# tyui592/Real_Time_Helmet_Detection

Measured on AMD Instinct MI355X. Metric: train imgs/sec, higher is better.
Workload: dtype bf16; 1 GPU; model=hourglass-1-ch128, global_batch=16, imsize=512, parallelism=dp1, engine=hip, fp8=False, hipgraph=True

## Files before the change

### real_time_helmet_detection_amd/ops/csrc/bindings.cpp

```cpp
#include <torch/extension.h>

namespace rthd {
torch::Tensor add_act_fwd(torch::Tensor a, torch::Tensor b, int64_t act);
torch::Tensor add_act_bwd(torch::Tensor dy, torch::Tensor y, int64_t act);

std::vector<torch::Tensor> pool2x2_fwd(torch::Tensor x, bool is_max,
                                       bool need_arg);
torch::Tensor pool2x2_bwd(torch::Tensor dy, torch::Tensor arg, bool is_max,
                          int64_t H, int64_t W);
std::vector<torch::Tensor> maxpool_same_fwd(torch::Tensor x, int64_t k,
                                            bool need_arg);
torch::Tensor maxpool_same_bwd(torch::Tensor dy, torch::Tensor arg,
                               int64_t k);

torch::Tensor upsample2x_add_fwd(torch::Tensor x,
                                 c10::optional<torch::Tensor> skip);
torch::Tensor upsample2x_bwd(torch::Tensor dy);

std::vector<torch::Tensor> centernet_loss_fwd(
    torch::Tensor phm, torch::Tensor poff, torch::Tensor psize,
    torch::Tensor ghm, torch::Tensor goff, torch::Tensor gsize,
    torch::Tensor mask, double alpha, double beta);
std::vector<torch::Tensor> centernet_loss_bwd(
    torch::Tensor phm, torch::Tensor poff, torch::Tensor psize,
    torch::Tensor ghm, torch::Tensor goff, torch::Tensor gsize,
    torch::Tensor mask, torch::Tensor sums, torch::Tensor gout,
    double alpha, double beta);
std::vector<torch::Tensor> centernet_loss_fused_fwd(
    torch::Tensor out, torch::Tensor ghm, torch::Tensor goff,
    torch::Tensor gsize, torch::Tensor mask, double alpha, double beta,
    bool sig_os);
torch::Tensor centernet_loss_fused_bwd(
    torch::Tensor out, torch::Tensor ghm, torch::Tensor goff,
    torch::Tensor gsize, torch::Tensor mask, torch::Tensor sums,
    torch::Tensor glosses, double alpha, double beta, bool sig_os);

std::vector<torch::Tensor> decode_fwd(torch::Tensor hm, torch::Tensor off,
                                      torch::Tensor wh, int64_t scale_factor,
                                      int64_t topk, int64_t pool_size,
                                      bool normalized);
std::vector<torch::Tensor> decode_logits(torch::Tensor out,
                                         int64_t scale_factor, int64_t topk,
                                         int64_t pool_size, bool normalized,
                                         bool flip);
torch::Tensor nms_fwd(torch::Tensor boxes, torch::Tensor scores,
                      double iou_threshold);
std::vector<torch::Tensor> nms_batched(torch::Tensor boxes,
                                       torch::Tensor scores,
                                       double iou_threshold,
                                       double conf_th);
std::vector<torch::Tensor> soft_nms_fwd(torch::Tensor boxes,
                                        torch::Tensor scores, double sigma,
                                        double score_th);
std::vector<torch::Tensor> soft_nms_batched(torch::Tensor boxes,
                                            torch::Tensor scores,
                                            double sigma, double score_th,
                                            double conf_th);

torch::Tensor pack_weights(torch::Tensor w, bool swap, bool to_bf16);
std::vector<torch::Tensor> pack_weights_pair(torch::Tensor w,
                                             bool to_bf16_fwd,
                                             bool to_bf16_dgrad);
torch::Tensor pack_weights_fp8(torch::Tensor w);
torch::Tensor conv_fwd_fp8r(torch::Tensor x, torch::Tensor wpk,
                            torch::Tensor scale, torch::Tensor shift,
                            c10::optional<torch::Tensor> skip,
                            int64_t KH, int64_t KW, int64_t stride,
                            int64_t pad, int64_t Cout, int64_t act,
                            bool out_fp8);
torch::Tensor conv_fwd(torch::Tensor x, torch::Tensor wpk,
                       torch::Tensor scale, torch::Tensor shift,
                       c10::optional<torch::Tensor> skip,
                       int64_t KH, int64_t KW, int64_t stride, int64_t pad,
                       int64_t Cout, int64_t act);
torch::Tensor conv_fwd_small(torch::Tensor x, torch::Tensor wpk,
                             torch::Tensor scale, torch::Tensor shift,
                             c10::optional<torch::Tensor> skip,
                             int64_t KH, int64_t KW, int64_t stride,
                             int64_t pad, int64_t Cout, int64_t act,
                             int64_t splitk);
torch::Tensor conv_fwd_k64(torch::Tensor x, torch::Tensor wpk,
                           torch::Tensor scale, torch::Tensor shift,
                           c10::optional<torch::Tensor> skip,
                           int64_t KH, int64_t KW, int64_t stride,
                           int64_t pad, int64_t Cout, int64_t act);
torch::Tensor stem_im2col(torch::Tensor x, int64_t KS, int64_t stride,
                          int64_t pad);
torch::Tensor wgrad(torch::Tensor x, torch::Tensor dy, int64_t KH,
                    int64_t KW, int64_t stride, int64_t pad);
torch::Tensor wgrad_bf16_fast(torch::Tensor x, torch::Tensor dy, int64_t KH,
                              int64_t KW, int64_t stride, int64_t pad,
                              const std::string& variant);
torch::Tensor lds_tr16_selftest();
std::string wgrad_bf16_choice(int64_t Cin, int64_t Cout, int64_t M);
int64_t wgrad_bf16_chunk_len(int64_t Cin, int64_t Cout, int64_t taps,
                             int64_t M);

std::vector<torch::Tensor> conv_fwd_stats(
    torch::Tensor x, torch::Tensor wpk, torch::Tensor scale,
    torch::Tensor shift, int64_t KH, int64_t KW, int64_t stride,
    int64_t pad, int64_t Cout, int64_t act);
std::vector<torch::Tensor> bn_stats_from_parts(
    torch::Tensor p1, torch::Tensor p2,
    c10::optional<torch::Tensor> running_mean,
    c10::optional<torch::Tensor> running_var,
    double momentum, double eps, int64_t M);
std::vector<torch::Tensor> bn_stats(torch::Tensor x,
                                    c10::optional<torch::Tensor> running_mean,
                                    c10::optional<torch::Tensor> running_var,
                                    double momentum, double eps);
torch::Tensor bn_act_fwd(torch::Tensor x, torch::Tensor mean,
                         torch::Tensor rstd, torch::Tensor gamma,
                         torch::Tensor beta, int64_t act,
                         c10::optional<torch::Tensor> skip);
std::vector<torch::Tensor> bn_act_bwd(torch::Tensor dy, torch::Tensor x,
                                      torch::Tensor mean, torch::Tensor rstd,
                                      torch::Tensor gamma, torch::Tensor beta,
                                      int64_t act,
                                      c10::optional<torch::Tensor> skip);
torch::Tensor col_sum(torch::Tensor x);

std::vector<torch::Tensor> encode_targets(torch::Tensor boxes,
                                          torch::Tensor labels, int64_t H,
                                          int64_t W, int64_t scale_factor,
                                          int64_t num_cls, bool normalized);
torch::Tensor normalize_u8(torch::Tensor img_u8, torch::Tensor table);
int64_t encode_chunk();
torch::Tensor augment_u8(torch::Tensor img_u8, torch::Tensor sizes,
                         torch::Tensor coef, int64_t T,
                         c10::optional<torch::Tensor> table);
}

PYBIND11_MODULE(TORCH_EXTENSION_NAME, m) {
  m.def("add_act_fwd", &rthd::add_act_fwd);
  m.def("add_act_bwd", &rthd::add_act_bwd);
  m.def("pool2x2_fwd", &rthd::pool2x2_fwd);
  m.def("pool2x2_bwd", &rthd::pool2x2_bwd);
  m.def("maxpool_same_fwd", &rthd::maxpool_same_fwd);
  m.def("maxpool_same_bwd", &rthd::maxpool_same_bwd);
  m.def("upsample2x_add_fwd", &rthd::upsample2x_add_fwd);
  m.def("upsample2x_bwd", &rthd::upsample2x_bwd);
  m.def("centernet_loss_fwd", &rthd::centernet_loss_fwd);
  m.def("centernet_loss_bwd", &rthd::centernet_loss_bwd);
  m.def("centernet_loss_fused_fwd", &rthd::centernet_loss_fused_fwd);
  m.def("centernet_loss_fused_bwd", &rthd::centernet_loss_fused_bwd);
  m.def("decode_fwd", &rthd::decode_fwd);
  m.def("decode_logits", &rthd::decode_logits);
  m.def("nms_fwd", &rthd::nms_fwd);
  m.def("nms_batched", &rthd::nms_batched);
  m.def("soft_nms", &rthd::soft_nms_fwd);
  m.def("soft_nms_batched", &rthd::soft_nms_batched);
  m.def("pack_weights",&rthd::pack_weights);
  m.def("pack_weights_pair", &rthd::pack_weights_pair);
  m.def("pack_weights_fp8", &rthd::pack_weights_fp8);
  m.def("conv_fwd_fp8r", &rthd::conv_fwd_fp8r);
  m.def("conv_fwd", &rthd::conv_fwd);
  m.def("conv_fwd_small", &rthd::conv_fwd_small);
  m.def("conv_fwd_k64", &rthd::conv_fwd_k64);
  m.def("stem_im2col", &rthd::stem_im2col);
  m.def("wgrad", &rthd::wgrad);
  m.def("wgrad_bf16_fast", &rthd::wgrad_bf16_fast,
        py::arg("x"), py::arg("dy"), py::arg("kh"), py::arg("kw"),
        py::arg("stride"), py::arg("pad"), py::arg("variant") = "");
  m.def("lds_tr16_selftest", &rthd::lds_tr16_selftest);
  m.def("wgrad_bf16_choice", &rthd::wgrad_bf16_choice);
  m.def("wgrad_bf16_chunk_len", &rthd::wgrad_bf16_chunk_len);
  m.def("conv_fwd_stats", &rthd::conv_fwd_stats);
  m.def("bn_stats_from_parts", &rthd::bn_stats_from_parts,
        py::arg("p1"), py::arg("p2"), py::arg("running_mean") = py::none(),
        py::arg("running_var") = py::none(), py::arg("momentum") = 0.1,
        py::arg("eps") = 1e-5, py::arg("m") = 1);
  m.def("bn_stats", &rthd::bn_stats);
  m.def("bn_act_fwd", &rthd::bn_act_fwd, py::arg("x"), py::arg("mean"), py::arg("rstd"), py::arg("gamma"), py::arg("beta"), py::arg("act"), py::arg("skip") = py::none());
  m.def("bn_act_bwd", &rthd::bn_act_bwd, py::arg("dy"), py::arg("x"), py::arg("mean"), py::arg("rstd"), py::arg("gamma"), py::arg("beta"), py::arg("act"), py::arg("skip") = py::none());
  m.def("col_sum", &rthd::col_sum);
  m.def("encode_targets", &rthd::encode_targets);
  m.def("normalize_u8", &rthd::normalize_u8);
  m.def("encode_chunk", &rthd::encode_chunk);
  m.def("augment_u8", &rthd::augment_u8, py::arg("img_u8"), py::arg("sizes"),
        py::arg("coef"), py::arg("T"), py::arg("table") = py::none());
}

namespace rthd {

static torch::Tensor maxpool2x2_op(torch::Tensor x) {
  return pool2x2_fwd(std::move(x), true, false)[0];
}
static torch::Tensor avgpool2x2_op(torch::Tensor x) {
  return pool2x2_fwd(std::move(x), false, false)[0];
}
static torch::Tensor maxpool_same_op(torch::Tensor x, int64_t k) {
  return maxpool_same_fwd(std::move(x), k, false)[0];
}
static std::tuple<torch::Tensor, torch::Tensor> nms_batched_op(
    torch::Tensor boxes, torch::Tensor scores, double iou, double conf) {
  auto v = nms_batched(std::move(boxes), std::move(scores), iou, conf);
  return {v[0], v[1]};
}
static std::tuple<torch::Tensor, torch::Tensor> soft_nms_op(
    torch::Tensor boxes, torch::Tensor scores, double sigma,
    double score_th) {
  auto v = soft_nms_fwd(std::move(boxes), std::move(scores), sigma, score_th);
  return {v[0], v[1]};
}
static std::tuple<torch::Tensor, torch::Tensor, torch::Tensor>
soft_nms_batched_op(torch::Tensor boxes, torch::Tensor scores, double sigma,
                    double score_th, double conf) {
  auto v = soft_nms_batched(std::move(boxes), std::move(scores), sigma,
                            score_th, conf);
  return {v[0], v[1], v[2]};
}
static std::tuple<torch::Tensor, torch::Tensor, torch::Tensor> decode_op(
    torch::Tensor hm, torch::Tensor off, torch::Tensor wh,
    int64_t scale_factor, int64_t topk, int64_t pool_size, bool normalized) {
  auto v = decode_fwd(std::move(hm), std::move(off), std::move(wh),
                      scale_factor, topk, pool_size, normalized);
  return {v[0], v[1], v[2]};
}
static std::tuple<torch::Tensor, torch::Tensor, torch::Tensor>
decode_logits_op(torch::Tensor out, int64_t scale_factor, int64_t topk,
                 int64_t pool_size, bool normalized, bool flip) {
  auto v = decode_logits(std::move(out), scale_factor, topk, pool_size,
                         normalized, flip);
  return {v[0], v[1], v[2]};
}

}

TORCH_LIBRARY(rthd, m) {
  m.def("conv_fwd(Tensor x, Tensor wpk, Tensor scale, Tensor shift, "
        "Tensor? skip, int kh, int kw, int stride, int pad, int cout, "
        "int act) -> Tensor");
  m.def("conv_fwd_fp8r(Tensor x, Tensor wpk, Tensor scale, Tensor shift, "
        "Tensor? skip, int kh, int kw, int stride, int pad, int cout, "
        "int act, bool out_fp8) -> Tensor");
  m.def("add_act_fwd(Tensor a, Tensor b, int act) -> Tensor");
  m.def("maxpool2x2(Tensor x) -> Tensor");
  m.def("avgpool2x2(Tensor x) -> Tensor");
  m.def("maxpool_same(Tensor x, int k) -> Tensor");
  m.def("upsample2x_add(Tensor x, Tensor? skip) -> Tensor");
  m.def("nms(Tensor boxes, Tensor scores, float iou) -> Tensor");
  m.def("nms_batched(Tensor boxes, Tensor scores, float iou, float conf) "
        "-> (Tensor, Tensor)");
  m.def("soft_nms(Tensor boxes, Tensor scores, float sigma, "
        "float score_th) -> (Tensor, Tensor)");
  m.def("soft_nms_batched(Tensor boxes, Tensor scores, float sigma, "
        "float score_th, float conf) -> (Tensor, Tensor, Tensor)");
  m.def("decode(Tensor hm, Tensor off, Tensor wh, int scale_factor, "
        "int topk, int pool_size, bool normalized) "
        "-> (Tensor, Tensor, Tensor)");
  m.def("decode_logits(Tensor out, int scale_factor, int topk, "
        "int pool_size, bool normalized, bool flip) "
        "-> (Tensor, Tensor, Tensor)");
  m.def("stem_im2col(Tensor x, int ks, int stride, int pad) -> Tensor");
}

TORCH_LIBRARY_IMPL(rthd, CUDA, m) {
  m.impl("conv_fwd", rthd::conv_fwd);
  m.impl("conv_fwd_fp8r", rthd::conv_fwd_fp8r);
  m.impl("add_act_fwd", rthd::add_act_fwd);
  m.impl("maxpool2x2", rthd::maxpool2x2_op);
  m.impl("avgpool2x2", rthd::avgpool2x2_op);
  m.impl("maxpool_same", rthd::maxpool_same_op);
  m.impl("upsample2x_add", rthd::upsample2x_add_fwd);
  m.impl("nms", rthd::nms_fwd);
  m.impl("nms_batched", rthd::nms_batched_op);
  m.impl("soft_nms", rthd::soft_nms_op);
  m.impl("soft_nms_batched", rthd::soft_nms_batched_op);
  m.impl("decode", rthd::decode_op);
  m.impl("decode_logits", rthd::decode_logits_op);
  m.impl("stem_im2col", rthd::stem_im2col);
}
```

### real_time_helmet_detection_amd/ops/csrc/conv.hip

```cpp
#include <mutex>
#include <type_traits>
#include <unordered_map>

#include "conv_common.h"

namespace rthd {



struct PackSrc {
  const float* w;
  int Cout, Cin, KH, KW;
  int64_t s0, s1, s2, s3;
};

template <typename T>
DEV_INLINE void pack_weight_elem(const PackSrc& a, T* __restrict__ pk,
                                 int64_t i, int Rows, int Rp, int Kp,
                                 int swap) {
  const int t = i / ((int64_t)Rp * Kp);
  const int row = (i / Kp) % Rp;
  const int k = i % Kp;
  float v = 0.f;
  const int Kdim = swap ? a.Cout : a.Cin;
// ... 81 lines not shown
        dim3(256), 0, s, pack_src(wc), pk.data_ptr<float>(), g.Rows, g.Rp,
        g.Kp, swap ? 1 : 0);
  HIP_CHECK_LAST();
  return pk;
}

std::vector<torch::Tensor> pack_weights_pair(torch::Tensor w,
                                             bool to_bf16_fwd,
                                             bool to_bf16_dgrad) {
  auto wc = w.to(at::kFloat);
  const PackGeo gf = pack_geo(wc, false), gd = pack_geo(wc, true);
  auto pk = pack_alloc(wc, gf, to_bf16_fwd);
  auto pkt = pack_alloc(wc, gd, to_bf16_dgrad);
  auto s = at::cuda::getCurrentCUDAStream();
  const dim3 grid(ew_grid(gf.n + gd.n, 256));
  auto launch = [&](auto* pf, auto* pd) {
    using TF = std::remove_pointer_t<decltype(pf)>;
    using TD = std::remove_pointer_t<decltype(pd)>;
    hipLaunchKernelGGL((pack_weights_pair_kernel<TF, TD>), grid, dim3(256),
        0, s, pack_src(wc), pf, pd, gf.Rp, gf.Kp, gd.Rp, gd.Kp);
  };
  bf16* fb = reinterpret_cast<bf16*>(pk.data_ptr());
  bf16* db = reinterpret_cast<bf16*>(pkt.data_ptr());
  float* ff = reinterpret_cast<float*>(pk.data_ptr());
  float* df = reinterpret_cast<float*>(pkt.data_ptr());
  if (to_bf16_fwd && to_bf16_dgrad) launch(fb, db);
  else if (to_bf16_fwd) launch(fb, df);
  else if (to_bf16_dgrad) launch(ff, db);
  else launch(ff, df);
  HIP_CHECK_LAST();
  return {pk, pkt};
}


DEV_INLINE int lds_off_f32(int row, int k) {
  return row * 128 + ((k ^ (row & 15)) << 2);
}

template <bool HAS_SKIP, bool STATS = false>
__global__ __launch_bounds__(256)
void conv_fwd_bf16_kernel(const bf16* __restrict__ x,
                          const bf16* __restrict__ wpk,
                          const float* __restrict__ scale,
                          const float* __restrict__ shift,
                          const bf16* __restrict__ skip,
                          const bf16* __restrict__ zpage,
                          bf16* __restrict__ y,
                          ConvGeo g, int act,
                          float* __restrict__ sp1 = nullptr,
                          float* __restrict__ sp2 = nullptr) {
  const int mblk = blockIdx.x;
  const int nblk = blockIdx.y;
  const int tid = threadIdx.x;
  const int lane = tid & 63;
  const int wid = tid >> 6;
  const int wr = wid >> 1, wc = wid & 1;

  extern __shared__ __attribute__((aligned(16))) char smem[];
  char* lds = smem;

  f32x4 acc[4][4] = {};

  const int st_row = tid >> 2;
  const int st_k8 = tid & 3;
  const int k8s0 = st_k8 ^ ((st_row >> 2) & 3);
  const int k8s1 = st_k8 ^ (((st_row + 64) >> 2) & 3);
  const int wbase = wid * 1024;

  int am[2], ab[2], ay[2], ax[2];
#pragma unroll
  for (int h = 0; h < 2; ++h) {
    am[h] = mblk * 128 + st_row + 64 * h;
    pixel_decompose(am[h], g, &ab[h], &ay[h], &ax[h]);
  }

  const int kc = g.Cinp / 32;
  const int taps = g.KH * g.KW;
  const int nsteps = taps * kc;

  int is_step = 0;
  int is_t = 0, is_kb = 0;
  const bf16* aptr[2];
  const bf16* bptr[2];
  bool avalid[2];
  auto tap_setup = [&]() {
    const int dy_ = is_t / g.KW - g.pad;
    const int dx_ = is_t % g.KW - g.pad;
#pragma unroll
    for (int h = 0; h < 2; ++h) {
      const int iy = ay[h] * g.stride + dy_;
      const int ix = ax[h] * g.stride + dx_;
      avalid[h] = am[h] < g.M && iy >= 0 && iy < g.H && ix >= 0 &&
                  ix < g.W;
      const int c0 = (h ? k8s1 : k8s0) * 8;
      aptr[h] = avalid[h]
          ? x + (((int64_t)ab[h] * g.H + iy) * g.W + ix) * g.Cin + c0
          : zpage;
    }
    bptr[0] = wpk + ((int64_t)is_t * g.Coutp + nblk * 128 + st_row) *
        g.Cinp + k8s0 * 8;
    bptr[1] = wpk + ((int64_t)is_t * g.Coutp + nblk * 128 + st_row + 64) *
        g.Cinp + k8s1 * 8;
  };
  tap_setup();

  auto issue_step = [&]() {
    char* base = lds + (is_step % 3) * 16384;
    const int cb = is_kb * 32;
    const bf16* a0 = (avalid[0] && cb + k8s0 * 8 < g.Cin) ? aptr[0] + cb
                                                          : zpage;
    const bf16* a1 = (avalid[1] && cb + k8s1 * 8 < g.Cin) ? aptr[1] + cb
                                                          : zpage;
    __builtin_amdgcn_global_load_lds((glb_void*)a0,
        (lds_void*)(base + wbase), 16, 0, 0);
    __builtin_amdgcn_global_load_lds((glb_void*)a1,
        (lds_void*)(base + 4096 + wbase), 16, 0, 0);
    __builtin_amdgcn_global_load_lds((glb_void*)(bptr[0] + cb),
        (lds_void*)(base + 8192 + wbase), 16, 0, 0);
    __builtin_amdgcn_global_load_lds((glb_void*)(bptr[1] + cb),
        (lds_void*)(base + 12288 + wbase), 16, 0, 0);
    ++is_step;
    if (++is_kb == kc) {
      is_kb = 0;
      if (++is_t < taps) tap_setup();
    }
  };

  issue_step();
  if (nsteps > 1) {
    issue_step();
    asm volatile("s_waitcnt vmcnt(%0)" ::"i"(4) : "memory");
  } else {
    asm volatile("s_waitcnt vmcnt(%0)" ::"i"(0) : "memory");
  }
  __builtin_amdgcn_s_barrier();

  for (int step = 0; step < nsteps; ++step) {
    char* A = lds + (step % 3) * 16384;
    char* B = A + 8192;
    if (step + 2 < nsteps) issue_step();

    const int arow_base = wr * 64 + (lane & 15);
    const int brow_base = wc * 64 + (lane & 15);
    const int k8 = lane >> 4;
    bf16x8 afrag[4], bfrag[4];
#pragma unroll
    for (int i = 0; i < 4; ++i) {
      afrag[i] = *reinterpret_cast<const bf16x8*>(
          A + lds_off_row64(arow_base + 16 * i, k8));
      bfrag[i] = *reinterpret_cast<const bf16x8*>(
          B + lds_off_row64(brow_base + 16 * i, k8));
    }
    asm volatile("s_setprio 1");
#pragma unroll
    for (int mi = 0; mi < 4; ++mi)
#pragma unroll
      for (int ni = 0; ni < 4; ++ni)
        acc[mi][ni] = __builtin_amdgcn_mfma_f32_16x16x32_bf16(
            afrag[mi], bfrag[ni], acc[mi][ni], 0, 0, 0);
    asm volatile("s_setprio 0");

    if (step + 2 < nsteps + 1) {
      if (step + 2 < nsteps)
        asm volatile("s_waitcnt vmcnt(%0)" ::"i"(4) : "memory");
      else
        asm volatile("s_waitcnt vmcnt(%0)" ::"i"(0) : "memory");
    }
    __builtin_amdgcn_s_barrier();
  }

  conv_epilogue<4, 4, HAS_SKIP, STATS>(
      acc, mblk * 128 + wr * 64, nblk * 128 + wc * 64 + (lane & 15), lane,
      g.M, g.Cout, scale, shift, skip, y, act, sp1, sp2,
      (int64_t)mblk * 2 + wr);
}

template <bool HAS_SKIP>
__global__ __launch_bounds__(256)
void conv_fwd_f32_kernel(const float* __restrict__ x,
                         const float* __restrict__ wpk,
                         const float* __restrict__ scale,
                         const float* __restrict__ shift,
                         const float* __restrict__ skip,
                         float* __restrict__ y,
                         ConvGeo g, int act) {
  const int mblk = blockIdx.x;
  const int nblk = blockIdx.y;
  const int tid = threadIdx.x;
  const int lane = tid & 63;
  const int wid = tid >> 6;
  const int wr = wid >> 1, wc = wid & 1;

  extern __shared__ __attribute__((aligned(16))) char smem[];
  float* ldsA = reinterpret_cast<float*>(smem);
  float* ldsB = reinterpret_cast<float*>(smem + 16384);

  f32x4 acc[4][4] = {};

  const int st_row = tid >> 2;
  const int st_k8 = (tid & 3) * 8;

  int am[2], ab[2], ayy[2], axx[2];
#pragma unroll
  for (int h = 0; h < 2; ++h) {
    am[h] = mblk * 128 + st_row + 64 * h;
    pixel_decompose(am[h], g, &ab[h], &ayy[h], &axx[h]);
  }

  const int nsteps = g.KH * g.KW * (g.Cinp / 32);
  const int kc_per_tap = g.Cinp / 32;

  for (int step = 0; step < nsteps; ++step) {
    const int t = step / kc_per_tap;
    const int kb = step % kc_per_tap;
    const int dy = t / g.KW - g.pad;
    const int dx = t % g.KW - g.pad;
    float* A = ldsA;
    float* B = ldsB;
    __syncthreads();

#pragma unroll
    for (int h = 0; h < 2; ++h) {
      const int iy = ayy[h] * g.stride + dy;
      const int ix = axx[h] * g.stride + dx;
      const int c0 = kb * 32 + st_k8;
      float v[8] = {};
      if (am[h] < g.M && iy >= 0 && iy < g.H && ix >= 0 && ix < g.W &&
          c0 < g.Cin) {
        const float* src =
            x + (((int64_t)ab[h] * g.H + iy) * g.W + ix) * g.Cin + c0;
#pragma unroll
        for (int e = 0; e < 8; ++e)
          v[e] = (c0 + e < g.Cin) ? src[e] : 0.f;
      }
#pragma unroll
      for (int e = 0; e < 8; ++e) {
        *reinterpret_cast<float*>(
            reinterpret_cast<char*>(A) +
            lds_off_f32(st_row + 64 * h, st_k8 + e)) = v[e];
      }
    }
#pragma unroll
    for (int h = 0; h < 2; ++h) {
      const int row = st_row + 64 * h;
      const int64_t src_off =
          ((int64_t)t * g.Coutp + nblk * 128 + row) * g.Cinp + kb * 32 +
          st_k8;
#pragma unroll
      for (int e = 0; e < 8; ++e) {
        *reinterpret_cast<float*>(
            reinterpret_cast<char*>(B) + lds_off_f32(row, st_k8 + e)) =
            wpk[src_off + e];
      }
    }

    __syncthreads();

    const int arow = wr * 64 + (lane & 15);
    const int brow = wc * 64 + (lane & 15);
    const int kl = lane >> 4;
#pragma unroll
    for (int ks = 0; ks < 8; ++ks) {
      float afrag[4], bfrag[4];
#pragma unroll
      for (int i = 0; i < 4; ++i) {
        afrag[i] = *reinterpret_cast<const float*>(
            reinterpret_cast<char*>(A) +
            lds_off_f32(arow + 16 * i, ks * 4 + kl));
        bfrag[i] = *reinterpret_cast<const float*>(
            reinterpret_cast<char*>(B) +
            lds_off_f32(brow + 16 * i, ks * 4 + kl));
      }
#pragma unroll
      for (int mi = 0; mi < 4; ++mi)
#pragma unroll
        for (int ni = 0; ni < 4; ++ni)
          acc[mi][ni] = __builtin_amdgcn_mfma_f32_16x16x4f32(
              afrag[mi], bfrag[ni], acc[mi][ni], 0, 0, 0);
    }

    __syncthreads();
  }

  conv_epilogue<4, 4, HAS_SKIP, false>(
      acc, mblk * 128 + wr * 64, nblk * 128 + wc * 64 + (lane & 15), lane,
      g.M, g.Cout, scale, shift, skip, y, act, nullptr, nullptr, 0);
}


const bf16* zero_page_bf16(const torch::Tensor& like) {
  static std::mutex mu;
  static std::unordered_map<int, torch::Tensor> pages;
  const int dev = like.device().index();
  std::lock_guard<std::mutex> lk(mu);
  auto it = pages.find(dev);
  if (it == pages.end())
    it = pages.emplace(dev, torch::zeros({8},
        like.options().dtype(at::kBFloat16))).first;
  return reinterpret_cast<const bf16*>(it->second.data_ptr());
}

namespace {

struct ConvChoice { int small; int splitk; };

std::mutex g_conv_tune_mu;
std::unordered_map<uint64_t, ConvChoice> g_conv_tune;

uint64_t conv_key(const ConvGeo& g) {
  uint64_t h = 1469598103934665603ull;
  auto mix = [&h](uint64_t v) {
    h ^= v + 0x9e3779b97f4a7c15ull + (h << 6) + (h >> 2);
  };
  mix(g.M); mix(g.Cin); mix(g.Cout); mix(g.KH); mix(g.KW); mix(g.stride);
  return h;
}

bool stream_capturing(hipStream_t s) {
  hipStreamCaptureStatus st = hipStreamCaptureStatusNone;
  if (hipStreamIsCapturing(s, &st) != hipSuccess) {
    (void)hipGetLastError();
    return true;
  }
  return st != hipStreamCaptureStatusNone;
}

template <typename F>
float time_usec(F&& fn, hipStream_t s) {
  hipEvent_t e0, e1;
  (void)hipEventCreate(&e0);
  (void)hipEventCreate(&e1);
  fn();
  float best = 1e30f;
  for (int r = 0; r < 3; ++r) {
    (void)hipEventRecord(e0, s);
    fn();
    (void)hipEventRecord(e1, s);
    (void)hipEventSynchronize(e1);
    float ms = 0.f;
    (void)hipEventElapsedTime(&ms, e0, e1);
    best = std::min(best, ms * 1000.f);
  }
  (void)hipEventDestroy(e0);
  (void)hipEventDestroy(e1);
  return best;
}

void launch_big(const ConvGeo& g, const ConvOperands& o, int act,
                float* p1, float* p2) {
  TORCH_CHECK(!(p1 && o.skip.defined()), "conv big: stats with skip");
  dim3 grid(cdiv(g.M, 128), g.Coutp / 128);
  auto s = at::cuda::getCurrentCUDAStream();
#define RTHD_BIG_LAUNCH(SKIP_, STATS_)                                     \
  hipLaunchKernelGGL((conv_fwd_bf16_kernel<SKIP_, STATS_>), grid,          \
      dim3(256), 3 * 16384, s, conv_ptr<const bf16>(o.x),                  \
      conv_ptr<const bf16>(o.wpk), o.scale.data_ptr<float>(),              \
      o.shift.data_ptr<float>(), conv_ptr<const bf16>(o.skip),             \
      zero_page_bf16(o.x), conv_ptr<bf16>(o.y), g, act, p1, p2)
  if (p1)                    RTHD_BIG_LAUNCH(false, true);
  else if (o.skip.defined()) RTHD_BIG_LAUNCH(true, false);
  else                       RTHD_BIG_LAUNCH(false, false);
#undef RTHD_BIG_LAUNCH
  HIP_CHECK_LAST();
}

ConvChoice choose_conv_variant(const ConvGeo& g, const ConvOperands& o,
                               int act) {
  const uint64_t key = conv_key(g);
  {
    std::lock_guard<std::mutex> lk(g_conv_tune_mu);
    auto it = g_conv_tune.find(key);
    if (it != g_conv_tune.end()) return it->second;
  }
  const int big_blocks = (int)cdiv(g.M, 128) * (g.Coutp / 128);
  const int nsteps = g.KH * g.KW * (g.Cinp / 32);
  const int base64 = (int)cdiv(g.M, 64) * (int)cdiv(g.Cout, 64);
  std::vector<int> cands;
  if (big_blocks < 512 || g.Cout <= 64) {
    for (int sk : {1, 2, 4, 8, 16}) {
      if (sk > 1 && (nsteps + sk - 1) / sk < 2) break;
      if ((int64_t)base64 * sk > 16384) break;
      cands.push_back(sk);
    }
  }
  ConvChoice ch{0, 1};
  auto s = at::cuda::getCurrentCUDAStream();
  if (stream_capturing(s) || getenv("RTHD_NO_AUTOTUNE")) {
    if (big_blocks >= 512 && g.Cout > 64) {
      ch = {0, 1};
    } else if (!cands.empty()) {
      ch = {1, cands.back()};
      for (int sk : cands) {
        if (base64 * sk >= 768) { ch = {1, sk}; break; }
      }
    }
  } else {
    float best = time_usec(
        [&] { launch_big(g, o, act, nullptr, nullptr); }, s.stream());
    const float tk = time_usec(
        [&] { launch_k64(g, o, act, nullptr, nullptr); }, s.stream());
    if (tk < best) { best = tk; ch = {2, 1}; }
    for (int sk : cands) {
      const float t = time_usec(
          [&] { launch_small(g, o, act, sk); }, s.stream());
      if (t < best) { best = t; ch = {1, sk}; }
    }
  }
  std::lock_guard<std::mutex> lk(g_conv_tune_mu);
  g_conv_tune[key] = ch;
  return ch;
}

}

torch::Tensor conv_fwd(torch::Tensor x, torch::Tensor wpk,
                       torch::Tensor scale, torch::Tensor shift,
                       c10::optional<torch::Tensor> skip,
                       int64_t KH, int64_t KW, int64_t stride, int64_t pad,
                       int64_t Cout, int64_t act) {
  const bool bf16_mode = wpk.scalar_type() == at::kBFloat16;
  TORCH_CHECK(bf16_mode || x.scalar_type() == at::kFloat,
              "f32 conv needs f32 input");
  const ConvGeo g = make_conv_geo("conv_fwd", x, wpk, KH, KW, stride, pad,
                                  Cout, 64);
  const auto dtype = bf16_mode ? at::kBFloat16 : at::kFloat;
  auto o = prep_conv_operands(g, x, wpk, scale, shift, skip, dtype, dtype);

  if (bf16_mode) {
    const ConvChoice ch = choose_conv_variant(g, o, (int)act);
    if (ch.small == 1)      launch_small(g, o, (int)act, ch.splitk);
    else if (ch.small == 2) launch_k64(g, o, (int)act, nullptr, nullptr);
    else                    launch_big(g, o, (int)act, nullptr, nullptr);
    return o.y;
  }

  dim3 grid(cdiv(g.M, 128), g.Coutp / 128);
  auto s = at::cuda::getCurrentCUDAStream();
  if (o.skip.defined())
    hipLaunchKernelGGL((conv_fwd_f32_kernel<true>), grid, dim3(256), 32768,
        s, o.x.data_ptr<float>(), wpk.data_ptr<float>(),
        o.scale.data_ptr<float>(), o.shift.data_ptr<float>(),
        o.skip.data_ptr<float>(), o.y.data_ptr<float>(), g, (int)act);
  else
    hipLaunchKernelGGL((conv_fwd_f32_kernel<false>), grid, dim3(256), 32768,
        s, o.x.data_ptr<float>(), wpk.data_ptr<float>(),
        o.scale.data_ptr<float>(), o.shift.data_ptr<float>(),
        (const float*)nullptr, o.y.data_ptr<float>(), g, (int)act);
  HIP_CHECK_LAST();
  return o.y;
}

std::vector<torch::Tensor> conv_fwd_stats(
    torch::Tensor x, torch::Tensor wpk, torch::Tensor scale,
    torch::Tensor shift, int64_t KH, int64_t KW, int64_t stride,
    int64_t pad, int64_t Cout, int64_t act) {
  TORCH_CHECK(wpk.scalar_type() == at::kBFloat16,
              "conv_fwd_stats: bf16 only (f32 path uses bn_stats)");
  const ConvGeo g = make_conv_geo("conv_fwd_stats", x, wpk, KH, KW, stride,
                                  pad, Cout, 64);
  auto o = prep_conv_operands(g, x, wpk, scale, shift, c10::nullopt,
                              at::kBFloat16, at::kBFloat16);
  const ConvChoice ch = choose_conv_variant(g, o, (int)act);
  if (ch.small == 1) {
    launch_small(g, o, (int)act, ch.splitk);
    return {o.y};
  }
  auto p1 = torch::empty({2 * cdiv(g.M, 128), Cout},
                         o.x.options().dtype(at::kFloat));
  auto p2 = torch::empty_like(p1);
  if (ch.small == 2)
    launch_k64(g, o, (int)act, p1.data_ptr<float>(), p2.data_ptr<float>());
  else
    launch_big(g, o, (int)act, p1.data_ptr<float>(), p2.data_ptr<float>());
  return {o.y, p1, p2};
}

}
```

### real_time_helmet_detection_amd/ops/csrc/conv_common.h

```cpp
#pragma once

#include <torch/extension.h>
#include <ATen/cuda/CUDAContext.h>

#include "common.h"

namespace rthd {

using bf16x8 = __attribute__((ext_vector_type(8))) short;
using f32x4 = __attribute__((ext_vector_type(4))) float;
using i32x8 = __attribute__((ext_vector_type(8))) int;

typedef __attribute__((address_space(3))) void lds_void;
typedef __attribute__((address_space(1))) const void glb_void;

struct ConvGeo {
  int B, H, W, Cin, Ho, Wo, Cout;
  int KH, KW, stride, pad;
  int Cinp;
  int Coutp;
  int M;
};


DEV_INLINE int lds_off_row64(int row, int k8) {
  return row * 64 + ((k8 ^ ((row >> 2) & 3)) << 4);
}
DEV_INLINE int lds_off_row128(int row, int chunk) {
  return row * 128 + ((chunk ^ (row & 7)) << 4);
}

DEV_INLINE void pixel_decompose(int m, const ConvGeo& g, int* b, int* y,
                                int* x) {
  const int mm = m < g.M ? m : 0;
  *b = mm / (g.Ho * g.Wo);
  const int r = mm % (g.Ho * g.Wo);
  *y = r / g.Wo;
  *x = r % g.Wo;
}

template <int MI, int NI, bool HAS_SKIP, bool STATS, typename OUT_T,
          typename SKIP_T>
DEV_INLINE void conv_epilogue(const f32x4 (&acc)[MI][NI], int row0, int col0,
                              int lane, int M, int Cout,
                              const float* __restrict__ scale,
                              const float* __restrict__ shift,
                              const SKIP_T* __restrict__ skip,
                              OUT_T* __restrict__ y, int act,
                              float* __restrict__ sp1,
                              float* __restrict__ sp2, int64_t chunk) {
  float esc[NI], esh[NI];
#pragma unroll
  for (int ni = 0; ni < NI; ++ni) {
    const int c = col0 + ni * 16;
    esc[ni] = c < Cout ? scale[c] : 0.f;
    esh[ni] = c < Cout ? shift[c] : 0.f;
  }
  const int row_in_frag = (lane >> 4) * 4;
  float s1[NI] = {}, s2[NI] = {};
#pragma unroll
  for (int mi = 0; mi < MI; ++mi) {
#pragma unroll
    for (int r = 0; r < 4; ++r) {
      const int m = row0 + mi * 16 + row_in_frag + r;
      if (m >= M) continue;
#pragma unroll
      for (int ni = 0; ni < NI; ++ni) {
        const int c = col0 + ni * 16;
        if (c >= Cout) continue;
        float v = acc[mi][ni][r];
        v = v * esc[ni] + esh[ni];
        if (HAS_SKIP) v += ldf(&skip[(int64_t)m * Cout + c]);
        v = apply_act(v, act);
        stf(&y[(int64_t)m * Cout + c], v);
        if (STATS) {
          s1[ni] += v;
          s2[ni] += v * v;
        }
      }
    }
  }
  if (STATS) {
#pragma unroll
    for (int ni = 0; ni < NI; ++ni) {
      float a = s1[ni], b = s2[ni];
      a += __shfl_xor(a, 16, 64);
      a += __shfl_xor(a, 32, 64);
      b += __shfl_xor(b, 16, 64);
      b += __shfl_xor(b, 32, 64);
      const int c = col0 + ni * 16;
      if ((lane >> 4) == 0 && c < Cout) {
        sp1[chunk * Cout + c] = a;
        sp2[chunk * Cout + c] = b;
      }
    }
  }
}

template <typename T, typename MMA>
DEV_INLINE void conv_mainloop_row128(const T* __restrict__ x,
                                     const T* __restrict__ wpk,
                                     const T* __restrict__ zpage,
                                     const ConvGeo& g, char* lds, int mblk,
                                     int nblk, int wid, int lane, MMA&& mma) {
  constexpr int EPC = 16 / (int)sizeof(T);
  constexpr int KSTEP = 8 * EPC;
  const int st_chunk = lane & 7;

  int am[4], ab[4], ay[4], ax[4], asw[4];
  const T* aptr[4];
  const T* bptr[4];
#pragma unroll
  for (int j = 0; j < 4; ++j) {
    const int row = (j * 4 + wid) * 8 + (lane >> 3);
    am[j] = mblk * 128 + row;
    asw[j] = (st_chunk ^ (row & 7)) * EPC;
    pixel_decompose(am[j], g, &ab[j], &ay[j], &ax[j]);
    bptr[j] = wpk + ((int64_t)nblk * 128 + row) * g.Cinp + asw[j];
  }

  const int kc = g.Cinp / KSTEP;
  const int taps = g.KH * g.KW;
  const int nsteps = taps * kc;
  const int64_t btap = (int64_t)g.Coutp * g.Cinp;

  int is_step = 0;
  int is_t = 0, is_kb = 0;
  bool avalid[4];
  auto tap_setup = [&]() {
    const int dy_ = is_t / g.KW - g.pad;
    const int dx_ = is_t % g.KW - g.pad;
#pragma unroll
    for (int j = 0; j < 4; ++j) {
      const int iy = ay[j] * g.stride + dy_;
      const int ix = ax[j] * g.stride + dx_;
      avalid[j] = am[j] < g.M && iy >= 0 && iy < g.H && ix >= 0 &&
                  ix < g.W;
      aptr[j] = avalid[j]
          ? x + (((int64_t)ab[j] * g.H + iy) * g.W + ix) * g.Cin + asw[j]
          : zpage;
    }
  };
  tap_setup();

  auto issue_step = [&]() {
    char* base = lds + (is_step & 1) * 32768;
    const int cb = is_kb * KSTEP;
    const int64_t boff = (int64_t)is_t * btap + cb;
#pragma unroll
    for (int j = 0; j < 4; ++j) {
      const T* a0 = (avalid[j] && cb + asw[j] < g.Cin) ? aptr[j] + cb : zpage;
      __builtin_amdgcn_global_load_lds((glb_void*)a0,
          (lds_void*)(base + (j * 4 + wid) * 1024 + (lane & 63) * 16),
          16, 0, 0);
      __builtin_amdgcn_global_load_lds((glb_void*)(bptr[j] + boff),
          (lds_void*)(base + 16384 + (j * 4 + wid) * 1024 +
                      (lane & 63) * 16), 16, 0, 0);
    }
    ++is_step;
    if (++is_kb == kc) {
      is_kb = 0;
      if (++is_t < taps) tap_setup();
    }
  };

  issue_step();
  asm volatile("s_waitcnt vmcnt(0)" ::: "memory");
  __builtin_amdgcn_s_barrier();

  for (int step = 0; step < nsteps; ++step) {
    char* A = lds + (step & 1) * 32768;
    char* B = A + 16384;
    if (step + 1 < nsteps) issue_step();

    mma(A, B);

    if (step + 1 < nsteps)
      asm volatile("s_waitcnt vmcnt(0)" ::: "memory");
    __builtin_amdgcn_s_barrier();
  }
}


inline ConvGeo make_conv_geo(const char* op, const torch::Tensor& x,
                             const torch::Tensor& wpk, int64_t KH,
                             int64_t KW, int64_t stride, int64_t pad,
                             int64_t Cout, int cin_pad) {
  ConvGeo g;
  g.B = x.size(0);
  g.Cin = x.size(1);
  g.H = x.size(2);
  g.W = x.size(3);
  g.KH = KH; g.KW = KW; g.stride = stride; g.pad = pad;
  g.Ho = (g.H + 2 * g.pad - (int)KH) / (int)stride + 1;
  g.Wo = (g.W + 2 * g.pad - (int)KW) / (int)stride + 1;
  g.Cout = Cout;
  g.Cinp = (int)cdiv(g.Cin, cin_pad) * cin_pad;
  g.Coutp = (int)cdiv(Cout, 128) * 128;
  g.M = g.B * g.Ho * g.Wo;
  TORCH_CHECK(g.Cin >= 1, op, ": bad Cin");
  TORCH_CHECK(wpk.scalar_type() == at::kFloat ||
              g.Cin % (cin_pad / 8) == 0,
              op, ": Cin % ", cin_pad / 8, " required, Cin=", g.Cin);
  TORCH_CHECK(wpk.size(0) == KH * KW && wpk.size(1) == g.Coutp &&
              wpk.size(2) == g.Cinp, op, ": packed weight shape");
  return g;
}

struct ConvOperands {
  torch::Tensor x, wpk, scale, shift, skip, y;
};

inline ConvOperands prep_conv_operands(
    const ConvGeo& g, const torch::Tensor& x, const torch::Tensor& wpk,
    const torch::Tensor& scale, const torch::Tensor& shift,
    const c10::optional<torch::Tensor>& skip, at::ScalarType io_dtype,
    at::ScalarType out_dtype) {
  ConvOperands o;
  o.wpk = wpk;
  o.x = x.contiguous(at::MemoryFormat::ChannelsLast);
  if (o.x.scalar_type() != io_dtype) o.x = o.x.to(io_dtype);
  o.scale = scale.to(at::kFloat).contiguous();
  o.shift = shift.to(at::kFloat).contiguous();
  if (skip.has_value())
    o.skip = skip->to(io_dtype).contiguous(at::MemoryFormat::ChannelsLast);
  o.y = torch::empty({g.B, (int64_t)g.Cout, g.Ho, g.Wo},
                     o.x.options().dtype(out_dtype)
                         .memory_format(at::MemoryFormat::ChannelsLast));
  return o;
}

template <typename T>
inline T* conv_ptr(const torch::Tensor& t) {
  return t.defined() ? reinterpret_cast<T*>(t.data_ptr()) : nullptr;
}

const bf16* zero_page_bf16(const torch::Tensor& like);

void launch_k64(const ConvGeo& g, const ConvOperands& o, int act,
                float* p1, float* p2);
void launch_small(const ConvGeo& g, const ConvOperands& o, int act,
                  int splitk);

torch::Tensor pack_weights(torch::Tensor w, bool swap, bool to_bf16);
std::vector<torch::Tensor> pack_weights_pair(torch::Tensor w,
                                             bool to_bf16_fwd,
                                             bool to_bf16_dgrad);
torch::Tensor pack_weights_fp8(torch::Tensor w);
torch::Tensor conv_fwd(torch::Tensor x, torch::Tensor wpk,
                       torch::Tensor scale, torch::Tensor shift,
                       c10::optional<torch::Tensor> skip,
                       int64_t KH, int64_t KW, int64_t stride, int64_t pad,
                       int64_t Cout, int64_t act);
std::vector<torch::Tensor> conv_fwd_stats(
    torch::Tensor x, torch::Tensor wpk, torch::Tensor scale,
    torch::Tensor shift, int64_t KH, int64_t KW, int64_t stride,
    int64_t pad, int64_t Cout, int64_t act);
torch::Tensor conv_fwd_k64(torch::Tensor x, torch::Tensor wpk,
                           torch::Tensor scale, torch::Tensor shift,
                           c10::optional<torch::Tensor> skip,
                           int64_t KH, int64_t KW, int64_t stride,
                           int64_t pad, int64_t Cout, int64_t act);
torch::Tensor conv_fwd_small(torch::Tensor x, torch::Tensor wpk,
                             torch::Tensor scale, torch::Tensor shift,
                             c10::optional<torch::Tensor> skip,
                             int64_t KH, int64_t KW, int64_t stride,
                             int64_t pad, int64_t Cout, int64_t act,
                             int64_t splitk);
torch::Tensor conv_fwd_fp8r(torch::Tensor x, torch::Tensor wpk,
                            torch::Tensor scale, torch::Tensor shift,
                            c10::optional<torch::Tensor> skip,
                            int64_t KH, int64_t KW, int64_t stride,
                            int64_t pad, int64_t Cout, int64_t act,
                            bool out_fp8);

}
```

Measured before the change: 1186 imgs/sec.

## Add halo-tiled implicit-GEMM 3x3 conv kernel with LDS-resident input patch

Adds a new forward conv kernel for 3x3 stride-1 convs with Cin 64/128. It loads an input spatial patch plus halo once into LDS and reuses it across all nine taps, while weights stream through a triple-buffered ring. The kernel is added to the autotuner and becomes the default choice under stream capture for large eligible convs. The aim is to cut redundant global reads of the im2col-style input. In exchange it needs a large LDS footprint, which may lower occupancy.

```diff
diff --git a/real_time_helmet_detection_amd/ops/csrc/bindings.cpp b/real_time_helmet_detection_amd/ops/csrc/bindings.cpp
--- a/real_time_helmet_detection_amd/ops/csrc/bindings.cpp
+++ b/real_time_helmet_detection_amd/ops/csrc/bindings.cpp
@@ -84,6 +84,11 @@
                            c10::optional<torch::Tensor> skip,
                            int64_t KH, int64_t KW, int64_t stride,
                            int64_t pad, int64_t Cout, int64_t act);
+torch::Tensor conv_fwd_halo(torch::Tensor x, torch::Tensor wpk,
+                            torch::Tensor scale, torch::Tensor shift,
+                            c10::optional<torch::Tensor> skip,
+                            int64_t KH, int64_t KW, int64_t stride,
+                            int64_t pad, int64_t Cout, int64_t act);
 torch::Tensor stem_im2col(torch::Tensor x, int64_t KS, int64_t stride,
                           int64_t pad);
 torch::Tensor wgrad(torch::Tensor x, torch::Tensor dy, int64_t KH,
@@ -157,6 +162,7 @@
   m.def("conv_fwd", &rthd::conv_fwd);
   m.def("conv_fwd_small", &rthd::conv_fwd_small);
   m.def("conv_fwd_k64", &rthd::conv_fwd_k64);
+  m.def("conv_fwd_halo", &rthd::conv_fwd_halo);
   m.def("stem_im2col", &rthd::stem_im2col);
   m.def("wgrad", &rthd::wgrad);
   m.def("wgrad_bf16_fast", &rthd::wgrad_bf16_fast,
diff --git a/real_time_helmet_detection_amd/ops/csrc/conv.hip b/real_time_helmet_detection_amd/ops/csrc/conv.hip
--- a/real_time_helmet_detection_amd/ops/csrc/conv.hip
+++ b/real_time_helmet_detection_amd/ops/csrc/conv.hip
@@ -407,7 +407,7 @@
 
 namespace {
 
-struct ConvChoice { int small; int splitk; };
+struct ConvChoice { int small; int splitk; int alt = 0; };
 
 std::mutex g_conv_tune_mu;
 std::unordered_map<uint64_t, ConvChoice> g_conv_tune;
@@ -418,6 +418,7 @@
     h ^= v + 0x9e3779b97f4a7c15ull + (h << 6) + (h >> 2);
   };
   mix(g.M); mix(g.Cin); mix(g.Cout); mix(g.KH); mix(g.KW); mix(g.stride);
+  mix(halo_eligible(g));
   return h;
 }
 
@@ -492,7 +493,8 @@
   auto s = at::cuda::getCurrentCUDAStream();
   if (stream_capturing(s) || getenv("RTHD_NO_AUTOTUNE")) {
     if (big_blocks >= 512 && g.Cout > 64) {
-      ch = {0, 1};
+      if (halo_eligible(g)) ch = {3, 1, 0};
+      else                  ch = {0, 1};
     } else if (!cands.empty()) {
       ch = {1, cands.back()};
       for (int sk : cands) {
@@ -505,10 +507,15 @@
     const float tk = time_usec(
         [&] { launch_k64(g, o, act, nullptr, nullptr); }, s.stream());
     if (tk < best) { best = tk; ch = {2, 1}; }
+    const int alt = ch.small;
     for (int sk : cands) {
       const float t = time_usec(
           [&] { launch_small(g, o, act, sk); }, s.stream());
       if (t < best) { best = t; ch = {1, sk}; }
+    }
+    if (halo_eligible(g)) {
+      const float t = time_usec([&] { launch_halo(g, o, act); }, s.stream());
+      if (t < best) { best = t; ch = {3, 1, alt}; }
     }
   }
   std::lock_guard<std::mutex> lk(g_conv_tune_mu);
@@ -535,6 +542,7 @@
     const ConvChoice ch = choose_conv_variant(g, o, (int)act);
     if (ch.small == 1)      launch_small(g, o, (int)act, ch.splitk);
     else if (ch.small == 2) launch_k64(g, o, (int)act, nullptr, nullptr);
+    else if (ch.small == 3) launch_halo(g, o, (int)act);
     else                    launch_big(g, o, (int)act, nullptr, nullptr);
     return o.y;
   }
@@ -573,7 +581,8 @@
   auto p1 = torch::empty({2 * cdiv(g.M, 128), Cout},
                          o.x.options().dtype(at::kFloat));
   auto p2 = torch::empty_like(p1);
-  if (ch.small == 2)
+  const int variant = ch.small == 3 ? ch.alt : ch.small;
+  if (variant == 2)
     launch_k64(g, o, (int)act, p1.data_ptr<float>(), p2.data_ptr<float>());
   else
     launch_big(g, o, (int)act, p1.data_ptr<float>(), p2.data_ptr<float>());
diff --git a/real_time_helmet_detection_amd/ops/csrc/conv_common.h b/real_time_helmet_detection_amd/ops/csrc/conv_common.h
--- a/real_time_helmet_detection_amd/ops/csrc/conv_common.h
+++ b/real_time_helmet_detection_amd/ops/csrc/conv_common.h
@@ -241,6 +241,8 @@
                 float* p1, float* p2);
 void launch_small(const ConvGeo& g, const ConvOperands& o, int act,
                   int splitk);
+bool halo_eligible(const ConvGeo& g);
+void launch_halo(const ConvGeo& g, const ConvOperands& o, int act);
 
 torch::Tensor pack_weights(torch::Tensor w, bool swap, bool to_bf16);
 std::vector<torch::Tensor> pack_weights_pair(torch::Tensor w,
@@ -261,6 +263,11 @@
                            c10::optional<torch::Tensor> skip,
                            int64_t KH, int64_t KW, int64_t stride,
                            int64_t pad, int64_t Cout, int64_t act);
+torch::Tensor conv_fwd_halo(torch::Tensor x, torch::Tensor wpk,
+                            torch::Tensor scale, torch::Tensor shift,
+                            c10::optional<torch::Tensor> skip,
+                            int64_t KH, int64_t KW, int64_t stride,
+                            int64_t pad, int64_t Cout, int64_t act);
 torch::Tensor conv_fwd_small(torch::Tensor x, torch::Tensor wpk,
                              torch::Tensor scale, torch::Tensor shift,
                              c10::optional<torch::Tensor> skip,
diff --git a/real_time_helmet_detection_amd/ops/csrc/conv_halo.hip b/real_time_helmet_detection_amd/ops/csrc/conv_halo.hip
--- /dev/null
+++ b/real_time_helmet_detection_amd/ops/csrc/conv_halo.hip
@@ -0,0 +1,301 @@
+#include <mutex>
+
+#include "conv_common.h"
+#include "conv_halo_geo.h"
+
+namespace rthd {
+
+namespace {
+
+typedef __attribute__((address_space(3))) char lds_char;
+
+template <int OFF>
+DEV_INLINE bf16x8 lds_read16(uint32_t addr) {
+  bf16x8 v;
+  asm volatile("ds_read_b128 %0, %1 offset:%2"
+               : "=v"(v) : "v"(addr), "n"(OFF) : "memory");
+  return v;
+}
+
+DEV_INLINE void wait_lgkm(int n) {
+  switch (n) {
+    case 0: asm volatile("s_waitcnt lgkmcnt(0)" ::: "memory"); break;
+    case 1: asm volatile("s_waitcnt lgkmcnt(1)" ::: "memory"); break;
+    case 2: asm volatile("s_waitcnt lgkmcnt(2)" ::: "memory"); break;
+    case 3: asm volatile("s_waitcnt lgkmcnt(3)" ::: "memory"); break;
+    case 4: asm volatile("s_waitcnt lgkmcnt(4)" ::: "memory"); break;
+    case 5: asm volatile("s_waitcnt lgkmcnt(5)" ::: "memory"); break;
+    case 6: asm volatile("s_waitcnt lgkmcnt(6)" ::: "memory"); break;
+    default: asm volatile("s_waitcnt lgkmcnt(7)" ::: "memory"); break;
+  }
+}
+
+template <int CIN, int MI, bool HAS_SKIP, bool WIDE>
+__global__ __launch_bounds__(256)
+void conv_halo_kernel(const bf16* __restrict__ x,
+                      const bf16* __restrict__ wpk,
+                      const float* __restrict__ scale,
+                      const float* __restrict__ shift,
+                      const bf16* __restrict__ skip,
+                      const bf16* __restrict__ zpage,
+                      bf16* __restrict__ y, HaloGeo g, int act) {
+  static_assert(!(HAS_SKIP && WIDE), "the wide epilogue has no skip input");
+  constexpr int TH = 2 * MI;
+  constexpr int RB = CIN * 2;
+  constexpr int KC = CIN / 32;
+  constexpr int NPIECE = ((TH + 2) * HALO_PW * RB + 1023) / 1024;
+  constexpr int PATCH_BYTES = NPIECE * 1024;
+  constexpr int NSTEPS = 9 * KC;
+  extern __shared__ __attribute__((aligned(16))) char smem[];
+  char* ring = smem + PATCH_BYTES;
+
+  const int tid = threadIdx.x;
+  const int lane = tid & 63;
+  const int wid = tid >> 6;
+  const int wr = wid >> 1, wc = wid & 1;
+
+  int nblk, b, ty0, tx0;
+  halo_cell_decompose(g, TH, blockIdx.x, &nblk, &b, &ty0, &tx0);
+
+#pragma unroll
+  for (int i = 0; i < (NPIECE + 3) / 4; ++i) {
+    const int f = i * 4 + wid;
+    if (f < NPIECE) {
+      int p, c;
+      halo_piece_slot(f, lane, RB, &p, &c);
+      const int64_t off = halo_src(g, TH, b, ty0, tx0, p, c);
+      const bf16* src = off < 0 ? zpage : x + off;
+      __builtin_amdgcn_global_load_lds((glb_void*)src,
+          (lds_void*)(smem + f * 1024), 16, 0, 0);
+    }
+  }
+
+  const int st_row = tid >> 2;
+  const int k8s = (tid & 3) ^ ((st_row >> 2) & 3);
+  const bf16* wp0 = wpk + ((int64_t)nblk * HALO_BN + st_row) * CIN + k8s * 8;
+  const bf16* wp1 = wp0 + 64 * CIN;
+  const int64_t wtap = (int64_t)g.Coutp * CIN;
+  auto issue_w = [&](int t, int kb, int buf) {
+    const int64_t o = t * wtap + kb * 32;
+    char* base = ring + buf * HALO_WSTAGE + wid * 1024;
+    __builtin_amdgcn_global_load_lds((glb_void*)(wp0 + o), (lds_void*)base,
+                                     16, 0, 0);
+    __builtin_amdgcn_global_load_lds((glb_void*)(wp1 + o),
+                                     (lds_void*)(base + 4096), 16, 0, 0);
+  };
+  issue_w(0, 0, 0);
+  issue_w(1 / KC, 1 % KC, 1);
+
+  const uint32_t lds0 = (uint32_t)(uintptr_t)(lds_char*)smem;
+  const uint32_t bbase =
+      lds0 + PATCH_BYTES + lds_off_row64(wc * 64 + (lane & 15), lane >> 4);
+
+  f32x4 acc[MI][4] = {};
+  int rbuf = 0;
+
+#pragma unroll 1
+  for (int t = 0; t < 9; ++t) {
+    const int dy = t / 3, dx = t - 3 * dy;
+    uint32_t aoff[MI];
+#pragma unroll
+    for (int mi = 0; mi < MI; ++mi)
+      aoff[mi] = halo_frag_off(wr * MI + mi, dy, dx, 0, lane, RB);
+
+#pragma unroll
+    for (int kb = 0; kb < KC; ++kb) {
+      if (t == 8 && kb == KC - 1)
+        asm volatile("s_waitcnt vmcnt(0)" ::: "memory");
+      else
+        asm volatile("s_waitcnt vmcnt(%0)" ::"n"(HALO_WPIECES) : "memory");
+      __builtin_amdgcn_s_barrier();
+
+      const uint32_t bb = bbase + rbuf * HALO_WSTAGE;
+      bf16x8 bfrag[4], afrag[MI];
+      bfrag[0] = lds_read16<0>(bb);
+      bfrag[1] = lds_read16<1024>(bb);
+      bfrag[2] = lds_read16<2048>(bb);
+      bfrag[3] = lds_read16<3072>(bb);
+#pragma unroll
+      for (int mi = 0; mi < MI; ++mi)
+        afrag[mi] = lds_read16<0>(lds0 + (aoff[mi] ^ (kb << 6)));
+
+      const int wbuf = rbuf == 0 ? 2 : rbuf - 1;
+      if (t * KC + kb + 2 < NSTEPS)
+        issue_w(t + (kb + 2) / KC, (kb + 2) % KC, wbuf);
+      rbuf = rbuf == 2 ? 0 : rbuf + 1;
+
+      __builtin_amdgcn_sched_barrier(0);
+      __builtin_amdgcn_s_setprio(1);
+#pragma unroll
+      for (int mi = 0; mi < MI; ++mi) {
+        wait_lgkm(MI - 1 - mi);
+        if (mi == 0) {
+#pragma unroll
+          for (int ni = 0; ni < 4; ++ni) asm volatile("" : "+v"(bfrag[ni]));
+        }
+        asm volatile("" : "+v"(afrag[mi]));
+        __builtin_amdgcn_sched_barrier(0);
+#pragma unroll
+        for (int ni = 0; ni < 4; ++ni)
+          acc[mi][ni] = __builtin_amdgcn_mfma_f32_16x16x32_bf16(
+              afrag[mi], bfrag[ni], acc[mi][ni], 0, 0, 0);
+        __builtin_amdgcn_sched_barrier(0);
+      }
+      __builtin_amdgcn_s_setprio(0);
+      __builtin_amdgcn_sched_barrier(0);
+    }
+  }
+
+  const int col0 = nblk * HALO_BN + wc * 64 + (lane & 15);
+  float esc[4], esh[4];
+#pragma unroll
+  for (int ni = 0; ni < 4; ++ni) {
+    const int c = col0 + ni * 16;
+    esc[ni] = c < g.Cout ? scale[c] : 0.f;
+    esh[ni] = c < g.Cout ? shift[c] : 0.f;
+  }
+  if (WIDE) {
+    __syncthreads();
+#pragma unroll
+    for (int mi = 0; mi < MI; ++mi) {
+#pragma unroll
+      for (int r = 0; r < 4; ++r) {
+        const int pl = (wr * MI + mi) * 16 + (lane >> 4) * 4 + r;
+#pragma unroll
+        for (int ni = 0; ni < 4; ++ni) {
+          const int cl = wc * 64 + ni * 16 + (lane & 15);
+          float v = acc[mi][ni][r];
+          v = v * esc[ni] + esh[ni];
+          v = apply_act(v, act);
+          const int chunk = (cl >> 3) ^ (((pl >> 2) & 3) << 1);
+          stf(reinterpret_cast<bf16*>(smem + pl * 256 + chunk * 16 +
+                                      (cl & 7) * 2), v);
+        }
+      }
+    }
+    __syncthreads();
+#pragma unroll
+    for (int i = 0; i < TH; ++i) {
+      const int idx = i * 256 + tid;
+      const int pl = idx >> 4, ch = idx & 15;
+      const int c = nblk * HALO_BN + ch * 8;
+      if (c >= g.Cout) continue;
+      const int chunk = ch ^ (((pl >> 2) & 3) << 1);
+      const bf16x8 v =
+          *reinterpret_cast<const bf16x8*>(smem + pl * 256 + chunk * 16);
+      const int64_t m =
+          ((int64_t)b * g.H + ty0 + (pl >> 4)) * g.W + tx0 + (pl & 15);
+      *reinterpret_cast<bf16x8*>(y + m * g.Cout + c) = v;
+    }
+  } else {
+#pragma unroll
+    for (int mi = 0; mi < MI; ++mi) {
+      const int64_t mrow =
+          ((int64_t)b * g.H + ty0 + wr * MI + mi) * g.W + tx0 +
+          (lane >> 4) * 4;
+#pragma unroll
+      for (int r = 0; r < 4; ++r) {
+        const int64_t m = mrow + r;
+#pragma unroll
+        for (int ni = 0; ni < 4; ++ni) {
+          const int c = col0 + ni * 16;
+          if (c >= g.Cout) continue;
+          float v = acc[mi][ni][r];
+          v = v * esc[ni] + esh[ni];
+          if (HAS_SKIP) v += ldf(&skip[m * g.Cout + c]);
+          v = apply_act(v, act);
+          stf(&y[m * g.Cout + c], v);
+        }
+      }
+    }
+  }
+}
+
+constexpr int HALO_MI = 4;
+constexpr int HALO_TH = 2 * HALO_MI;
+
+constexpr int halo_lds_bytes(int CIN, int MI) {
+  return ((2 * MI + 2) * HALO_PW * CIN * 2 + 1023) / 1024 * 1024 +
+         HALO_NBUF * HALO_WSTAGE;
+}
+
+template <int CIN, int MI, bool HAS_SKIP, bool WIDE>
+void halo_launch_inst(const HaloGeo& hg, const ConvOperands& o, int act) {
+  constexpr int lds = halo_lds_bytes(CIN, MI);
+  static_assert(!WIDE || lds >= 2 * MI * 16 * 256,
+                "the output tile must fit in the LDS of the main loop");
+  auto* kern = &conv_halo_kernel<CIN, MI, HAS_SKIP, WIDE>;
+  if (lds > 65536) {
+    static std::mutex mu;
+    static uint64_t done = 0;
+    int dev = 0;
+    TORCH_CHECK(hipGetDevice(&dev) == hipSuccess && dev < 64,
+                "conv_halo: bad device");
+    std::lock_guard<std::mutex> lk(mu);
+    if (!((done >> dev) & 1)) {
+      const hipError_t e = hipFuncSetAttribute(
+          reinterpret_cast<const void*>(kern),
+          hipFuncAttributeMaxDynamicSharedMemorySize, lds);
+      TORCH_CHECK(e == hipSuccess, "conv_halo: cannot opt in to ", lds,
+                  " B of LDS: ", hipGetErrorString(e));
+      done |= (uint64_t)1 << dev;
+    }
+  }
+  const dim3 grid((unsigned)(hg.B * hg.tiles_y * hg.tiles_x *
+                             (hg.Coutp / HALO_BN)));
+  hipLaunchKernelGGL(kern, grid, dim3(256), lds,
+      at::cuda::getCurrentCUDAStream(), conv_ptr<const bf16>(o.x),
+      conv_ptr<const bf16>(o.wpk), o.scale.data_ptr<float>(),
+      o.shift.data_ptr<float>(), conv_ptr<const bf16>(o.skip),
+      zero_page_bf16(o.x), conv_ptr<bf16>(o.y), hg, act);
+}
+
+template <int CIN>
+void halo_launch_cin(const HaloGeo& hg, const ConvOperands& o, int act) {
+  if (o.skip.defined())
+    halo_launch_inst<CIN, HALO_MI, true, false>(hg, o, act);
+  else if (hg.Cout % 8 == 0)
+    halo_launch_inst<CIN, HALO_MI, false, true>(hg, o, act);
+  else
+    halo_launch_inst<CIN, HALO_MI, false, false>(hg, o, act);
+}
+
+}
+
+bool halo_eligible(const ConvGeo& g) {
+  return g.KH == 3 && g.KW == 3 && g.stride == 1 && g.pad == 1 &&
+         (g.Cin == 64 || g.Cin == 128) && g.Cinp == g.Cin &&
+         g.H % HALO_TH == 0 && g.W % HALO_TW == 0;
+}
+
+void launch_halo(const ConvGeo& g, const ConvOperands& o, int act) {
+  TORCH_CHECK(halo_eligible(g), "conv_halo: needs 3x3 stride 1 pad 1, Cin "
+              "64 or 128, H % ", HALO_TH, " == 0 and W % ", HALO_TW,
+              " == 0; got k", g.KH, "x", g.KW, " s", g.stride, " p", g.pad,
+              " Cin ", g.Cin, " H ", g.H, " W ", g.W);
+  HaloGeo hg;
+  hg.B = g.B; hg.H = g.H; hg.W = g.W; hg.Cin = g.Cin;
+  hg.Cout = g.Cout; hg.Coutp = g.Coutp;
+  hg.tiles_y = g.H / HALO_TH;
+  hg.tiles_x = g.W / HALO_TW;
+  if (g.Cin == 128) halo_launch_cin<128>(hg, o, act);
+  else              halo_launch_cin<64>(hg, o, act);
+  HIP_CHECK_LAST();
+}
+
+torch::Tensor conv_fwd_halo(torch::Tensor x, torch::Tensor wpk,
+                            torch::Tensor scale, torch::Tensor shift,
+                            c10::optional<torch::Tensor> skip,
+                            int64_t KH, int64_t KW, int64_t stride,
+                            int64_t pad, int64_t Cout, int64_t act) {
+  TORCH_CHECK(wpk.scalar_type() == at::kBFloat16,
+              "conv_fwd_halo: bf16 packed weights required");
+  const ConvGeo g = make_conv_geo("conv_fwd_halo", x, wpk, KH, KW, stride,
+                                  pad, Cout, 64);
+  auto o = prep_conv_operands(g, x, wpk, scale, shift, skip, at::kBFloat16,
+                              at::kBFloat16);
+  launch_halo(g, o, (int)act);
+  return o.y;
+}
+
+}
diff --git a/real_time_helmet_detection_amd/ops/csrc/conv_halo_geo.h b/real_time_helmet_detection_amd/ops/csrc/conv_halo_geo.h
--- /dev/null
+++ b/real_time_helmet_detection_amd/ops/csrc/conv_halo_geo.h
@@ -0,0 +1,83 @@
+#pragma once
+
+#include <cstdint>
+
+#if defined(__HIPCC__)
+#define HALO_HD __host__ __device__ inline
+#else
+#define HALO_HD inline
+#endif
+
+namespace rthd {
+
+constexpr int HALO_TW = 16;
+constexpr int HALO_PW = HALO_TW + 2;
+constexpr int HALO_BN = 128;
+constexpr int HALO_WSTAGE = HALO_BN * 64;
+constexpr int HALO_NBUF = 3;
+constexpr int HALO_WPIECES = 2;
+
+struct HaloGeo {
+  int B, H, W, Cin, Cout, Coutp;
+  int tiles_y, tiles_x;
+};
+
+HALO_HD int halo_patch_px(int TH) { return (TH + 2) * HALO_PW; }
+
+HALO_HD int halo_patch_pieces(int TH, int RB) {
+  return (halo_patch_px(TH) * RB + 1023) / 1024;
+}
+
+HALO_HD int halo_swz(int p, int RB) {
+  return RB == 256 ? ((p & 7) << 1) : (((p >> 1) & 3) << 1);
+}
+
+HALO_HD int halo_lds_off(int p, int chunk, int RB) {
+  return p * RB + ((chunk ^ halo_swz(p, RB)) << 4);
+}
+
+HALO_HD int halo_piece_byte(int f, int lane) { return f * 1024 + lane * 16; }
+
+HALO_HD void halo_piece_slot(int f, int lane, int RB, int* p, int* chunk) {
+  const int byte = halo_piece_byte(f, lane);
+  const int q = byte / RB;
+  *p = q;
+  *chunk = ((byte % RB) >> 4) ^ halo_swz(q, RB);
+}
+
+HALO_HD int64_t halo_src(const HaloGeo& g, int TH, int b, int ty0, int tx0,
+                         int p, int chunk) {
+  const int py = p / HALO_PW, px = p - py * HALO_PW;
+  const int iy = ty0 - 1 + py, ix = tx0 - 1 + px;
+  const bool ok = (p < halo_patch_px(TH)) & (iy >= 0) & (iy < g.H) &
+                  (ix >= 0) & (ix < g.W);
+  const int64_t off =
+      ((int64_t)(b * g.H + iy) * g.W + ix) * g.Cin + chunk * 8;
+  return ok ? off : -1;
+}
+
+HALO_HD int halo_frag_px(int r, int dy, int dx) {
+  return (r + dy) * HALO_PW + dx;
+}
+
+HALO_HD int halo_frag_off(int r, int dy, int dx, int kb, int lane, int RB) {
+  const int p = halo_frag_px(r, dy, dx) + (lane & 15);
+  return halo_lds_off(p, 4 * kb + (lane >> 4), RB);
+}
+
+HALO_HD void halo_cell_decompose(const HaloGeo& g, int TH, int cell,
+                                 int* nblk, int* b, int* ty0, int* tx0) {
+  const int nn = g.Coutp / HALO_BN;
+  *nblk = cell % nn;
+  int t = cell / nn;
+  *tx0 = (t % g.tiles_x) * HALO_TW;
+  t /= g.tiles_x;
+  *ty0 = (t % g.tiles_y) * TH;
+  *b = t / g.tiles_y;
+}
+
+HALO_HD int halo_wait_count(int step, int nsteps) {
+  return step + 1 < nsteps ? HALO_WPIECES : 0;
+}
+
+}
```

Measured after the change: 1298 imgs/sec, median of 6. 1.1x the previous value.
